# solonas13/REAL

Hardware: AMD Instinct MI355X
Metric: aligned reads/sec (100 bp, k≤3) at 1/2/4/8 MI355X; achieved HBM GB/s vs peak (higher is better)
Workload: dtype u64

## Files before the change

### real_amd/csrc/index_build.hip

```cpp
#include "real_hip_internal.h"

#include <cstring>
#include <rocprim/device/device_radix_sort.hpp>
#include <rocprim/device/device_scan.hpp>
#include <rocprim/iterator/transform_iterator.hpp>
#include <rocprim/device/device_select.hpp>
#include <rocprim/iterator/counting_iterator.hpp>

__global__ void pack_text_kernel(const uint8_t *__restrict__ sym, uint64_t n, uint64_t *__restrict__ text,
                                 uint64_t *__restrict__ wild, unsigned long long *n_wild)
{
    uint64_t w = (uint64_t)blockIdx.x * blockDim.x + threadIdx.x;
    uint64_t base = w * 64;
    if (base >= n) return;
    uint64_t t0 = 0, t1 = 0, wd = 0;
    for (int b = 0; b < 64; ++b) {
        uint64_t i = base + b;
        if (i < n) {
            uint64_t c = sym[i];
            if (c > 3) wd |= 1ull << (63 - b);
            c &= 3;
            if (b < 32) t0 |= c << (62 - 2 * b); else t1 |= c << (62 - 2 * (b - 32));
        }
    }
// ... 213 lines not shown
        if (!complex_ && c > 15) {
            uint32_t cnt[16];
            bucket_groups(ent, start, end, pbits, fbits >= 32 ? 15u : (1u << fbits) - 1, cnt);
#pragma unroll
            for (int g = 0; g < 16; ++g) complex_ = complex_ || cnt[g] > 15;
        }
        out = complex_ ? c : 0u;
    }
    ovf_cnt[p] = out;
}

__global__ void rows_fill_kernel(const uint32_t *__restrict__ bkt, const uint2 *__restrict__ ent, uint64_t nbuckets, uint32_t pbits,
                                 uint32_t fbits, const uint32_t *__restrict__ ovf_start, uint4 *__restrict__ rows, uint2 *__restrict__ ovf)
{
    const uint64_t p = (uint64_t)blockIdx.x * blockDim.x + threadIdx.x;
    if (p >= nbuckets) return;
    const uint32_t start = bkt[p], end = bkt[p + 1], c = end - start;
    const uint32_t os = ovf_start[p], oc = ovf_start[p + 1] - os;
    uint32_t w[32];
#pragma unroll
    for (int i = 0; i < 32; ++i) w[i] = 0;
    uint32_t cnt[16];
    bucket_groups(ent, start, end, pbits, fbits >= 32 ? 15u : (1u << fbits) - 1, cnt);
    if (oc) {
        rh_row_set_complex(w, os, c);
#pragma unroll
        for (int g = 0; g < 16; ++g) rh_row_set_count8(w, g, cnt[g]);
        for (uint32_t j = 0; j < c; ++j) ovf[os + j] = ent[start + j];
    } else {
#pragma unroll
        for (int g = 0; g < 16; ++g) rh_row_set_count4(w, g, cnt[g]);
        const uint32_t p16 = pbits < 16 ? pbits : 16;
        const uint32_t pmask = pbits ? ((1u << pbits) - 1) : 0u;
        for (uint32_t j = 0; j < c; ++j) {
            const uint2 e = ent[start + j];
            const uint32_t key = pbits ? ((e.x & pmask) >> (pbits - p16)) : rh_fp16(e.x);
            const uint32_t hw[3] = {key & 0xffffu, e.y & 0xffffu, e.y >> 16};
#pragma unroll
            for (int t = 0; t < 3; ++t) {
                const uint32_t h = rh_row_entry_hw(j) + t;
                const uint32_t v = hw[t] << (16 * (h & 1));
#pragma unroll
                for (int i = 2; i < 32; ++i) if ((h >> 1) == (uint32_t)i) w[i] |= v;
            }
        }
    }
#pragma unroll
    for (int i = 0; i < 8; ++i) rows[p * 8 + i] = make_uint4(w[4 * i], w[4 * i + 1], w[4 * i + 2], w[4 * i + 3]);
}

__device__ __forceinline__ uint32_t row_entries(uint32_t h0, uint32_t h1, uint32_t w3) { return rh_row_complex(h0, h1) ? w3 : rh_row_group4(h0, h1, 16).x; }

__global__ void pair_overflow_kernel(const uint32_t *__restrict__ bkt, const uint2 *__restrict__ ent, uint64_t nbuckets, uint32_t pbits,
                                     uint32_t gbits, const uint4 *__restrict__ rows, uint32_t *__restrict__ ovf_cnt)
{
    const uint64_t p = (uint64_t)blockIdx.x * blockDim.x + threadIdx.x;
    if (p > nbuckets) return;
    uint32_t out = 0;
    if (p < nbuckets) {
        const uint4 h = rows[p * 8];
        const uint32_t ca = row_entries(h.x, h.y, h.w);
        const uint32_t start = bkt[p], end = bkt[p + 1], c = end - start;
        bool complex_ = rh_row_complex(h.x, h.y) || ca + c > RH_ROW_CAP;
        if (!complex_ && c > 15) {
            uint32_t cnt[16];
            bucket_groups(ent, start, end, pbits, (1u << gbits) - 1, cnt);
#pragma unroll
            for (int g = 0; g < 16; ++g) complex_ = complex_ || cnt[g] > 15;
        }
        out = complex_ ? ca + c : 0u;
    }
    ovf_cnt[p] = out;
}

__global__ void pair_fill_kernel(const uint32_t *__restrict__ bkt, const uint2 *__restrict__ ent, uint64_t nbuckets, uint32_t pbits,
                                 uint32_t gbits, const uint32_t *__restrict__ ovf_start, uint32_t *rows, const uint2 *__restrict__ first_ovf,
                                 uint2 *__restrict__ ovf, const uint64_t *__restrict__ T, uint32_t l, int first_list)
{
// ... 4 lines not shown
    if (!c && !oc) return;
    uint32_t *w = rows + p * 32;
    const uint32_t h0 = w[0], h1 = w[1];
    const bool first_complex = rh_row_complex(h0, h1);
    const uint32_t ca = row_entries(h0, h1, w[3]);
    uint32_t cnt[16];
    bucket_groups(ent, start, end, pbits, (1u << gbits) - 1, cnt);
    if (oc) {
        uint32_t hd[8] = {0, 0, 0, 0, 0, 0, 0, 0};
        rh_row_set_complex(hd, os, ca + c);
        if (first_complex) {
            const uint32_t fo = w[2];
            for (int i = 4; i < 8; ++i) hd[i] = w[i];
            for (uint32_t j = 0; j < ca; ++j) ovf[os + j] = first_ovf[fo + j];
        } else {
            uint32_t j = 0;
            for (uint32_t g = 0; g < 16; ++g) {
                const uint32_t cg = rh_row_group4(h0, h1, g).y;
                rh_row_set_count8(hd, g, cg);
                for (uint32_t i = 0; i < cg; ++i, ++j) {
                    const uint32_t wp = rh_row_entry(w, j).y;
                    const uint32_t partner = (uint32_t)(window_signature(T, wp, l, 5 - first_list) >> (l - pbits));
                    ovf[os + j] = make_uint2((g << pbits) | partner, wp);
                }
            }
        }
        for (uint32_t g = 0; g < 16; ++g) if (cnt[g]) rh_row_set_count8(hd, g, cnt[g]);
        for (uint32_t j = 0; j < c; ++j) ovf[os + ca + j] = ent[start + j];
        for (int i = 0; i < 32; ++i) w[i] = i < 8 ? hd[i] : 0u;
    } else {
        uint32_t hd[2] = {h0, h1};
        for (uint32_t g = 0; g < 16; ++g) rh_row_set_count4(hd, g, cnt[g]);
        w[0] = hd[0]; w[1] = hd[1];
        uint16_t *hw = reinterpret_cast<uint16_t *>(w);
        const uint32_t p16 = pbits < 16 ? pbits : 16, pmask = (1u << pbits) - 1;
        for (uint32_t j = 0; j < c; ++j) {
            const uint2 e = ent[start + j];
            const uint32_t h = rh_row_entry_hw(ca + j);
            hw[h] = (uint16_t)((e.x & pmask) >> (pbits - p16)); hw[h + 1] = (uint16_t)(e.y & 0xffffu); hw[h + 2] = (uint16_t)(e.y >> 16);
        }
    }
}

__device__ __forceinline__ uint32_t ovf_groups_below(const uint2 *__restrict__ ovf, uint32_t o0, uint32_t tot, uint32_t pbits, uint32_t g)
{
    if (g == 0) return 0;
    if (g >= 16) return tot;
    uint32_t x = 0, y = tot;
    while (x < y) { const uint32_t mid = x + ((y - x) >> 1); if ((ovf[o0 + mid].x >> pbits) < g) x = mid + 1; else y = mid; }
    return x;
}
__global__ void rows_sizes_kernel(const uint4 *__restrict__ rows, const uint2 *__restrict__ ovf, uint64_t nbuckets, uint32_t pbits, uint32_t g0,
                                  uint32_t g1, uint32_t *__restrict__ size)
{
    const uint64_t p = (uint64_t)blockIdx.x * blockDim.x + threadIdx.x;
    if (p > nbuckets) return;
    uint32_t c = 0;
    if (p < nbuckets) {
        const uint4 h = rows[p * 8];
        c = rh_row_complex(h.x, h.y) ? ovf_groups_below(ovf, h.z, h.w, pbits, g1) - ovf_groups_below(ovf, h.z, h.w, pbits, g0)
                                     : rh_row_group4(h.x, h.y, g1).x - rh_row_group4(h.x, h.y, g0).x;
    }
    size[p] = c;
}
__global__ void rows_unpack_kernel(const uint4 *__restrict__ rows, const uint2 *__restrict__ ovf, uint64_t nbuckets, uint32_t pbits, uint32_t g0,
                                   const uint32_t *__restrict__ off, uint2 *__restrict__ out)
{
    const uint64_t p = (uint64_t)blockIdx.x * blockDim.x + threadIdx.x;
    if (p >= nbuckets) return;
    const uint32_t *w = reinterpret_cast<const uint32_t *>(rows + p * 8);
    const uint32_t o = off[p], c = off[p + 1] - o;
    if (rh_row_complex(w[0], w[1])) {
// ... 658 lines not shown
```

### real_amd/csrc/match_kernel.hip

```cpp
#include "match_common.h"

#ifndef RH_ABLATE
#define RH_ABLATE 0
#endif
#ifndef RH_PHASE_TIMING
#define RH_PHASE_TIMING 0
#endif

#if RH_PHASE_TIMING
#define PH_NOW() ((unsigned)__builtin_amdgcn_s_memrealtime())
#else
#define PH_NOW() 0u
#endif
#define EB 8
#define MQ 16
#define QUEUE_BYTES (MQ * 64u * 5u + 6u * 64u * 4u)
enum : int { TK_STARTS = 0, TK_DIRECTORY = 1, TK_ROWS = 3, TK_ROWS_WIDE = 4 };
__host__ __device__ constexpr uint32_t stg_bytes(int W, int TK) { return TK >= TK_ROWS ? 11008u : (W <= 4 ? QUEUE_BYTES : 9728u); }
#define MQR 8u
static_assert(MQR == RH_QSPILL_SLOTS, "the spill area holds a second queue of MQR slots per lane");
#define NPEND2 24
#define MQR2 24u
#define STG_PAD 16u
#ifndef RH_KEEP_TW_MAXW
// ... 572 lines not shown
{
    const uintptr_t a0 = (uintptr_t)src, a1 = a0 + nbytes, c0 = a0 & ~(uintptr_t)15;
    for (uintptr_t c = c0 + 16u * lane; c < a1; c += 16u * 64u) {
        const uint32_t lo = STG_PAD + (uint32_t)(c - c0);
        if (c >= a0 && c + 16 <= a1) {
            *reinterpret_cast<uint4 *>(stg + lo) = *reinterpret_cast<const uint4 *>(c);
        } else {
            for (int b = 0; b < 16; ++b)
                if (c + b >= a0 && c + b < a1) stg[lo + b] = *reinterpret_cast<const uint8_t *>(c + b);
        }
    }
    return STG_PAD + (uint32_t)(a0 - c0);
}
__device__ __forceinline__ void wave_lds_sync()
{
    __builtin_amdgcn_fence(__ATOMIC_SEQ_CST, "wavefront");
    __builtin_amdgcn_wave_barrier();
}

template <class T>
__device__ __forceinline__ bool quals_ahead(const MatchArgs &a, uint64_t o0, uint64_t o1, const uint8_t *&src, uint32_t &nbytes, uint32_t &late, uint32_t &skew)
{
    if (!a.b.qual || a.b.gl < 64) return false;
    const uint64_t gb = __shfl(o0, 0), ge = __shfl(o1, 63);
    skew = (uint32_t)((uintptr_t)(a.b.qual + gb) & 15u);
    src = a.b.qual + gb - skew;
    nbytes = (uint32_t)(ge - gb) + skew;
    late = nbytes <= 64u * 128u ? 0u : T::ROWBUF - STG_PAD;
    return ge >= gb && gb >= skew && ge - gb + skew <= T::STG_CAP;
}
template <class T>
__device__ __forceinline__ uint32_t quals_at(uint32_t late, uint32_t skew) { return (late ? STG_PAD : T::ROWBUF) + skew; }

__device__ __forceinline__ void quals_landed()
{
    asm volatile("s_waitcnt vmcnt(0)" ::: "memory");
}

template <class T, int LA0, int LA1>
__device__ __forceinline__ void match_lists_rows(const MatchArgs &a, LaneState<T> &s, const double *sLL, uint8_t *stg, bool act, bool qlast)
{
    constexpr bool wide = T::WIDE;
    constexpr int NL = LA1 - LA0;
    uint32_t lane = threadIdx.x & 63;
    asm volatile("" : "+v"(lane));
    uint32_t *q_pos = reinterpret_cast<uint32_t *>(stg) + lane;
    uint8_t *q_la = stg + T::QSLOTS * 64 * 4 + lane;
    uint8_t *rowbuf = stg + T::ROWBUF;
    const uint32_t bb = a.b_bits;
    const uint32_t gbits = a.ix.fbits, pbits = a.ix.pbits, p16 = pbits < 16 ? pbits : 16;
    const uint32_t pmask = (1u << pbits) - 1;
    uint64_t M = 0, MA = 0, MB = 0;
    if (!wide) {
        const uint32_t mb = (1u << bb) - 1;
        M = ((uint64_t)(uint32_t)(s.shi >> bb) << 48) | ((uint64_t)((uint32_t)s.shi & mb) << 32) | ((uint64_t)(uint32_t)(s.slo >> bb) << 16) |
            (uint64_t)((uint32_t)s.slo & mb);
    } else {
        const uint64_t mb = (bb >= 32) ? 0xffffffffull : ((1ull << bb) - 1);
        MA = ((s.shi >> bb) << 32) | (s.shi & mb);
        MB = ((s.slo >> bb) << 32) | (s.slo & mb);
    }
    auto sig_of = [&](int la) {
        const uint2 x = rh_list_segs(la);
        return (((uint32_t)(M >> (48 - 16 * x.x)) & 0xffffu) << bb) | ((uint32_t)(M >> (48 - 16 * x.y)) & 0xffffu);
    };
    auto sig_wide = [&](int la) {
// ... 104 lines not shown
                    if ((g >> 2) == (uint32_t)q) e_cnt = (w >> (8 * (g & 3))) & 255u;
                    const uint32_t y = ~w | ~upto;
                    sat255 |= (y - 0x01010101u) & ~y & 0x80808080u;
                }
                const bool sat = sat255 != 0;
                const uint32_t o0 = row(2), tot = row(3);
                e_base = o0 + off;
                if (sat) {
                    const uint2 kr = key_group_range(a.ix.ent[la], o0, o0 + tot, wide ? 28u : pbits, g);
                    e_base = kr.x; e_cnt = kr.y;
                }
            }
            if (!wide) s.addC(e_cnt);
            s.addP(e_cnt);
            if (e_cnt > T::BIG) { s.p_n = PEND_OVF; s.cslot = (!T::PASS2 && T::HAS_PASS2 && e_cnt <= BIG_T2) ? SLOT_NONE : SLOT_BIG; e_cnt = 0; }
            if (RH_ABLATE & 4) e_cnt = 0;
        }
        const uint32_t rk = wide ? rh_fp16(r) : (r >> (pbits - p16));
        U64x2 pre = {0ull, 0ull};
        if (e_ovf && e_cnt) pre = load2(reinterpret_cast<const uint64_t *>(a.ix.ent[la] + e_base));
        if (li + 1 < NL) ISSUE_ROWS(la + 1);
        auto take = [&](bool pass, uint32_t pos) {
            const bool merge = pass && qn && pos == q_last;
            if ((!wide || T::DEFER) && pass && !merge && qn >= 2) {
                for (uint32_t k = 0; k + 1 < qn; ++k)
                    if (q_pos[k * 64] == pos) { q_la[k * 64] |= (uint8_t)(1u << la); pass = false; break; }
            }
            if (pass && !merge && qn == T::QSLOTS) { s.p_n = PEND_OVF; e_cnt = 0; pass = false; }
            const uint32_t slot = merge ? qn - 1 : qn;
            const uint32_t lav = (merge ? q_lastla : 0u) | (1u << la);
            if (pass) { q_pos[slot * 64] = pos; q_la[slot * 64] = (uint8_t)lav; q_last = pos; q_lastla = lav; qn = slot + 1; }
        };
        auto passes = [&](uint32_t x) { return wide ? (x == 0u) : (__popc(((x >> 1) | x) & 0x55555555u) <= a.seedkmax); };
        uint32_t passm = 0;
        while (__any(!e_ovf && e_j < e_cnt)) {
#pragma unroll
            for (uint32_t u = 0; u < 4; ++u) {
                const uint32_t jj = e_j + u;
                const bool ok = !e_ovf && jj < e_cnt;
                const uint32_t h = ok ? rh_row_entry_hw(e_base + jj) : 4u;
                const uint32_t d0 = row(h >> 1);
                const uint32_t key = (h & 1) ? (d0 >> 16) : (d0 & 0xffffu);
                passm |= (ok && passes(key ^ rk) ? 1u : 0u) << (jj & 31u);
            }
            e_j += 4;
        }
        if (!T::PASS2 && T::HAS_PASS2 && __popc(passm) > NPEND) { s.p_n = PEND_OVF; passm = 0; e_cnt = 0; }
        while (__any(passm != 0)) {
            const bool step = passm != 0;
            const uint32_t jj = step ? (uint32_t)__ffs((int)passm) - 1u : 0u;
            passm &= passm - 1u;
            const uint32_t h = step ? rh_row_entry_hw(e_base + jj) : 4u;
            const uint32_t d0 = row(h >> 1), d1 = row((h >> 1) + 1);
            take(step, (h & 1) ? d1 : ((d0 >> 16) | (d1 << 16)));
        }
        auto take_ovf = [&](bool ok, uint2 e) { take(ok && passes(wide ? (e.x ^ r) : ((e.x & pmask) ^ r)), e.y); };
        if (__any(e_ovf && e_cnt)) {
            take_ovf(e_ovf && e_cnt > 0, make_uint2((uint32_t)pre.a, (uint32_t)(pre.a >> 32)));
            take_ovf(e_ovf && e_cnt > 1, make_uint2((uint32_t)pre.b, (uint32_t)(pre.b >> 32)));
        }
        e_j = 2;
        while (__any(e_ovf && e_j < e_cnt)) {
            uint2 e[T::OVN];
#pragma unroll
            for (uint32_t u = 0; u < T::OVN; ++u) e[u] = (e_ovf && e_j + u < e_cnt) ? a.ix.ent[la][e_base + e_j + u] : make_uint2(0u, 0u);
#pragma unroll
            for (uint32_t u = 0; u < T::OVN; ++u) take_ovf(e_ovf && e_j + u < e_cnt, e[u]);
            e_j += T::OVN;
        }
#if RH_PHASE_TIMING
        s.tD += PH_NOW() - ph1;
#endif
    }
    if (T::SCORES && qlast) ISSUE_QUALS();
#if RH_PHASE_TIMING
    const unsigned ph2 = PH_NOW();
#endif
    if (s.p_n == PEND_OVF) qn = 0;
    {
        CandText<T::W> c0;
        uint32_t rp0 = qn ? q_pos[0] : 0u;
        if (qn) cand_load(a, s, rp0, c0);
        for (uint32_t k = 0; k < qn; ++k) {
            CandText<T::W> c1;
            uint32_t rp1 = 0;
            if (k + 1 < qn) { rp1 = q_pos[(k + 1) * 64]; cand_load(a, s, rp1, c1); }
            process_loaded(a, s, sLL, rp0, (uint32_t)q_la[k * 64], c0);
            c0 = c1; rp0 = rp1;
        }
    }
#if RH_PHASE_TIMING
    s.tR += PH_NOW() - ph2;
#endif
    if (T::SCORES && qlast) ISSUE_QUALS_LATE();
#undef ISSUE_QUALS
#undef ISSUE_QUALS_LATE
#undef QUAL_DMA
}

template <class T>
__device__ __forceinline__ void match_rows_paired(const MatchArgs &a, LaneState<T> &s, const double *sLL, uint8_t *stg, bool act, uint32_t rhi,
                                                  uint32_t rlo)
{
    constexpr uint32_t QS = T::QSLOTS;
    uint32_t lane = threadIdx.x & 63;
    asm volatile("" : "+v"(lane));
    uint32_t *q_pos = reinterpret_cast<uint32_t *>(stg) + lane;
    uint8_t *q_la = stg + QS * 64 * 4 + lane;
    uint8_t *rowbuf = stg + T::ROWBUF;
    auto spill = [&](uint32_t k) -> uint2 & { return a.qspill[((size_t)(blockIdx.x * 4u + (threadIdx.x >> 6)) * QS + (k - QS)) * 64u + lane]; };
    const uint32_t bb = a.b_bits;
    const uint32_t gbits = a.ix.fbits, pbits = a.ix.pbits, p16 = pbits < 16 ? pbits : 16;
    const uint32_t pmask = (1u << pbits) - 1;
    const uint32_t mb = (1u << bb) - 1, fhi = (uint32_t)s.shi, flo = (uint32_t)s.slo;
    auto sig_of = [&](uint32_t strand, uint32_t la) {
        const uint32_t hi = strand ? rhi : fhi, lo = strand ? rlo : flo;
        const uint2 x = rh_list_segs(la);
        const uint32_t sa_ = ((x.x < 2 ? hi : lo) >> ((x.x & 1) ? 0u : bb)) & mb, sc_ = ((x.y < 2 ? hi : lo) >> ((x.y & 1) ? 0u : bb)) & mb;
        return (sa_ << bb) | sc_;
    };
    auto row_of = [&](uint32_t li) { return rh_row_addr(li >> 1, sig_of(li & 1u, li >> 1), a.l, gbits).row; };
    uint32_t qn = 0, qnf = 0, q_last = 0, q_lastla = 0;
    auto q_getp = [&](uint32_t k) { return k < QS ? q_pos[k * 64] : spill(k).x; };
    auto q_getl = [&](uint32_t k) { return k < QS ? (uint32_t)q_la[k * 64] : spill(k).y; };
    uint4 va0, va1, va2, va3, va4, va5, va6, va7;
    uint32_t *bkx = reinterpret_cast<uint32_t *>(stg + T::BKX);
#define ISSUE_ROWS_P(LI)                                                                                                    \
    do {                                                                                                                    \
        bkx[(lane & 7) * 8 + (lane >> 3)] = act ? row_of(LI) : 0u;                                                          \
        __builtin_amdgcn_wave_barrier();                                                                                    \
        const uint4 b0_ = *reinterpret_cast<const uint4 *>(bkx + (lane >> 3) * 8);                                          \
        const uint4 b1_ = *reinterpret_cast<const uint4 *>(bkx + (lane >> 3) * 8 + 4);                                      \
        const uint4 *__restrict__ R_ = reinterpret_cast<const uint4 *>(a.ix.bkt[(LI) >> 1]) + (lane & 7);                   \
        va0 = R_[(uint64_t)b0_.x * 8]; va1 = R_[(uint64_t)b0_.y * 8]; va2 = R_[(uint64_t)b0_.z * 8];                        \
        va3 = R_[(uint64_t)b0_.w * 8]; va4 = R_[(uint64_t)b1_.x * 8]; va5 = R_[(uint64_t)b1_.y * 8];                        \
        va6 = R_[(uint64_t)b1_.z * 8]; va7 = R_[(uint64_t)b1_.w * 8];                                                       \
    } while (0)
#define QUAL_DMA(SRC_OFF, LDS_ADDR, NBYTES, NCHUNK)                                                                                           \
    _Pragma("unroll") for (uint32_t i = 0; i < (NCHUNK); ++i)                                                                                 \
        if (16u * lane + 1024u * i + 16u <= (NBYTES)) {                                                                                       \
            const uint8_t *g_ = qsrc + (SRC_OFF) + 16u * lane + 1024u * i;                                                                    \
            uint32_t keep_;                                                                                                                   \
            asm volatile("s_mov_b32 %0, m0\n\ts_mov_b32 m0, %2\n\ts_nop 0\n\tglobal_load_lds_dwordx4 %1, off\n\ts_mov_b32 m0, %0"         \
                         : "=&s"(keep_) : "v"(g_), "s"((LDS_ADDR) + 1024u * i) : "memory");                                                   \
        }
    ISSUE_ROWS_P(0u);
#pragma unroll 1
    for (uint32_t li = 0; li < 8; ++li) {
        const uint32_t tbl = li >> 1, ks = li & 1u;
#if RH_PHASE_TIMING
        const unsigned ph0 = PH_NOW();
#endif
        wave_lds_sync();
        {
            uint8_t *d = rowbuf + (lane >> 3) * 128 + (((lane & 7) ^ ((lane >> 3) & 7)) * 16);
            *reinterpret_cast<uint4 *>(d + 0 * 1024) = va0; *reinterpret_cast<uint4 *>(d + 1 * 1024) = va1;
            *reinterpret_cast<uint4 *>(d + 2 * 1024) = va2; *reinterpret_cast<uint4 *>(d + 3 * 1024) = va3;
            *reinterpret_cast<uint4 *>(d + 4 * 1024) = va4; *reinterpret_cast<uint4 *>(d + 5 * 1024) = va5;
            *reinterpret_cast<uint4 *>(d + 6 * 1024) = va6; *reinterpret_cast<uint4 *>(d + 7 * 1024) = va7;
        }
        wave_lds_sync();
#if RH_PHASE_TIMING
        unsigned ph1 = PH_NOW();
        s.tW += ph1 - ph0;
#endif
        const uint8_t *rowb = rowbuf + lane * 128;
        const uint32_t sw = lane & 7;
        auto row = [&](uint32_t d) { return *reinterpret_cast<const uint32_t *>(rowb + ((((d >> 2) ^ sw) << 4) | ((d & 3) << 2))); };
        const RhRowAddr ra = rh_row_addr(tbl, sig_of(ks, tbl), a.l, gbits);
        const uint32_t nhalf = tbl < 2 ? 2u : 1u;
#pragma unroll 1
        for (uint32_t half = 0; half < nhalf; ++half) {
            const uint32_t strand = ks ^ half, la = half ? 5 - tbl : tbl;
            const uint32_t g = ra.group | (half << (gbits - 1));
            const uint32_t r = sig_of(strand, 5 - la) >> (a.l - pbits);
            const bool mine = act && !(s.p_n == PEND_OVF) && !(RH_ABLATE & 8);
            uint32_t e_cnt = 0, e_j = 0, e_base = 0;
            bool e_ovf = false;
            if (mine) {
                s.addL(1u);
                const uint32_t h0 = row(0), h1 = row(1);
                if (!rh_row_complex(h0, h1)) {
                    e_cnt = ((g < 8 ? h0 : h1) >> (4 * (g & 7))) & 15u;
                    const uint32_t m0 = g < 8 ? (g ? (h0 & (0xffffffffu >> (32 - 4 * g))) : 0u) : h0;
                    const uint32_t m1 = g > 8 ? (h1 & (0xffffffffu >> (32 - 4 * (g - 8)))) : 0u;
                    const uint32_t b0 = (m0 & 0x0f0f0f0fu) + ((m0 >> 4) & 0x0f0f0f0fu), b1 = (m1 & 0x0f0f0f0fu) + ((m1 >> 4) & 0x0f0f0f0fu);
                    e_base = __builtin_amdgcn_sad_u8(b0, 0u, __builtin_amdgcn_sad_u8(b1, 0u, 0u));
                } else {
                    e_ovf = true;
                    uint32_t off = 0, sat255 = 0;
#pragma unroll
                    for (int q = 0; q < 4; ++q) {
                        const uint32_t w = row(4 + q);
                        const int nb = (int)g - 4 * q;
                        const uint32_t below = nb <= 0 ? 0u : (nb >= 4 ? 0xffffffffu : ((1u << (8 * nb)) - 1u));
                        const uint32_t upto = nb < 0 ? 0u : (nb >= 3 ? 0xffffffffu : ((1u << (8 * (nb + 1))) - 1u));
                        off = __builtin_amdgcn_sad_u8(w & below, 0u, off);
                        if ((g >> 2) == (uint32_t)q) e_cnt = (w >> (8 * (g & 3))) & 255u;
                        const uint32_t y = ~w | ~upto;
                        sat255 |= (y - 0x01010101u) & ~y & 0x80808080u;
                    }
                    const uint32_t o0 = row(2), tot = row(3);
                    e_base = o0 + off;
                    if (sat255 != 0) {
                        const uint2 kr = key_group_range(a.ix.ent[tbl], o0, o0 + tot, pbits, g);
                        e_base = kr.x; e_cnt = kr.y;
                    }
                }
                s.addC(e_cnt);
                s.addP(e_cnt);
                if (e_cnt > T::BIG) { s.p_n = PEND_OVF; s.cslot = e_cnt <= BIG_T2 ? SLOT_NONE : SLOT_BIG; e_cnt = 0; }
                if (RH_ABLATE & 4) e_cnt = 0;
            }
            U64x2 pre = {0ull, 0ull};
            if (e_ovf && e_cnt) pre = load2(reinterpret_cast<const uint64_t *>(a.ix.ent[tbl] + e_base));
            if (half == 0 && li + 1 < 8) ISSUE_ROWS_P(li + 1);
            auto take = [&](bool pass, uint32_t pos) {
                const bool merge = pass && qn && pos == q_last && (q_lastla >> 6) == strand;
                if (pass && !merge && qn >= 2) {
                    for (uint32_t k = 0; k + 1 < qn; ++k)
                        if (q_getp(k) == pos && (q_getl(k) >> 6) == strand) {
                            if (k < QS) q_la[k * 64] |= (uint8_t)(1u << la); else spill(k).y |= 1u << la;
                            pass = false; break;
                        }
                }
                if (pass && !merge && (strand ? qn - qnf : qnf) == QS) { s.p_n = PEND_OVF; e_cnt = 0; pass = false; }
                const uint32_t slot = merge ? qn - 1 : qn;
                const uint32_t lav = (merge ? q_lastla : (strand << 6)) | (1u << la);
                if (pass) {
                    if (slot < QS) { q_pos[slot * 64] = pos; q_la[slot * 64] = (uint8_t)lav; } else spill(slot) = make_uint2(pos, lav);
                    q_last = pos; q_lastla = lav; qn = slot + 1;
                    if (!merge && !strand) qnf++;
                }
            };
            auto passes = [&](uint32_t x) { return __popc(((x >> 1) | x) & 0x55555555u) <= a.seedkmax; };
            uint32_t passm = 0;
            while (__any(!e_ovf && e_j < e_cnt)) {
#pragma unroll
                for (uint32_t u = 0; u < 4; ++u) {
                    const uint32_t jj = e_j + u;
                    const bool ok = !e_ovf && jj < e_cnt;
                    const uint32_t h = ok ? rh_row_entry_hw(e_base + jj) : 4u;
                    const uint32_t d0 = row(h >> 1);
                    const uint32_t key = (h & 1) ? (d0 >> 16) : (d0 & 0xffffu);
                    passm |= (ok && passes(key ^ (r >> (pbits - p16))) ? 1u : 0u) << (jj & 31u);
                }
                e_j += 4;
            }
            if (__popc(passm) > NPEND) { s.p_n = PEND_OVF; passm = 0; e_cnt = 0; }
            while (__any(passm != 0)) {
                const bool step = passm != 0;
                const uint32_t jj = step ? (uint32_t)__ffs((int)passm) - 1u : 0u;
                passm &= passm - 1u;
                const uint32_t h = step ? rh_row_entry_hw(e_base + jj) : 4u;
                const uint32_t d0 = row(h >> 1), d1 = row((h >> 1) + 1);
                take(step, (h & 1) ? d1 : ((d0 >> 16) | (d1 << 16)));
            }
            auto take_ovf = [&](bool ok, uint2 e) { take(ok && passes((e.x & pmask) ^ r), e.y); };
            if (__any(e_ovf && e_cnt)) {
                take_ovf(e_ovf && e_cnt > 0, make_uint2((uint32_t)pre.a, (uint32_t)(pre.a >> 32)));
                take_ovf(e_ovf && e_cnt > 1, make_uint2((uint32_t)pre.b, (uint32_t)(pre.b >> 32)));
            }
            e_j = 2;
            while (__any(e_ovf && e_j < e_cnt)) {
                uint2 e[T::OVN];
#pragma unroll
                for (uint32_t u = 0; u < T::OVN; ++u) e[u] = (e_ovf && e_j + u < e_cnt) ? a.ix.ent[tbl][e_base + e_j + u] : make_uint2(0u, 0u);
#pragma unroll
                for (uint32_t u = 0; u < T::OVN; ++u) take_ovf(e_ovf && e_j + u < e_cnt, e[u]);
                e_j += T::OVN;
            }
        }
#if RH_PHASE_TIMING
        s.tD += PH_NOW() - ph1;
#endif
    }
    const uint32_t patl = act ? s.patl : 32u * T::W;
#pragma unroll 1
    for (uint32_t inv = 0; inv < 2; ++inv) {
        if (inv && act) {
            uint64_t R[T::W];
            revcomp_words<T::W>(s.O, R, patl);
#pragma unroll
            for (int j = 0; j < T::W; ++j) s.O[j] = R[j];
        }
        s.shi = inv ? rhi : fhi; s.slo = inv ? rlo : flo;
        s.reset_strand((int)inv);
        if (T::SCORES && inv) {
            const uint8_t *qsrc;
            uint32_t qbytes, qlate, qskew;
            if (quals_ahead<T>(a, s.o0, s.o1, qsrc, qbytes, qlate, qskew)) {
// ... 321 lines not shown
```

### real_amd/csrc/real_hip_internal.h

```cpp
#pragma once

#include <hip/hip_runtime.h>
#include <stdint.h>
#include <string>
#include <vector>

#include "real_hip.h"

#define RH_MAXW 10
static_assert(RH_MAXW * 32 == REAL_HIP_MAX_PATL, "one lane-per-read instance per 32 bases up to REAL_HIP_MAX_PATL");
#define RH_CSTRIPES 1024
#define RH_QSPILL_SLOTS 8u

struct DevText {
    const uint64_t *text;
    const uint64_t *wild;
    const uint64_t *frag_start;
    uint64_t n;
    uint32_t n_frag;
    uint32_t has_wild;
    uint32_t fileid;
};

enum RhLayout : uint32_t { RH_LAYOUT_STARTS = 0, RH_LAYOUT_DIGEST = 1, RH_LAYOUT_FINGERPRINT = 2, RH_LAYOUT_ROWS = 3 };
// ... 18 lines not shown
#define RH_FP_SLOTS 8u
static inline __host__ __device__ uint32_t rh_fp11(uint32_t key) { return (key * 0x9E3779B1u) >> 21; }

static inline __host__ __device__ uint2 key_group_range(const uint2 *E, uint32_t lo, uint32_t hi, uint32_t shift, uint32_t key)
{
    uint32_t x = lo, y = hi;
    while (x < y) { const uint32_t mid = x + ((y - x) >> 1); if ((E[mid].x >> shift) < key) x = mid + 1; else y = mid; }
    const uint32_t first = x;
    for (y = hi; x < y;) { const uint32_t mid = x + ((y - x) >> 1); if ((E[mid].x >> shift) <= key) x = mid + 1; else y = mid; }
    return make_uint2(first, x - first);
}

#define RH_ROW_CAP 20u
#define RH_ROW_SAT 255u
static inline __host__ __device__ uint32_t rh_fp16(uint32_t key) { return ((key & 0x0fffffffu) * 0x9E3779B1u) >> 16; }
static inline __host__ __device__ bool rh_row_complex(uint32_t h0, uint32_t h1) { return (h0 & h1) == 0xffffffffu; }
static inline __host__ __device__ uint2 rh_row_group4(uint32_t h0, uint32_t h1, uint32_t g)
{
    uint32_t base = 0, cnt = 0;
    for (uint32_t q = 0; q < 16; ++q) { const uint32_t c = ((q < 8 ? h0 : h1) >> (4 * (q & 7))) & 15u; if (q < g) base += c; if (q == g) cnt = c; }
    return make_uint2(base, cnt);
}
static inline __host__ __device__ uint2 rh_row_group8(const uint32_t *row, uint32_t g, bool *sat)
{
    uint32_t base = 0, cnt = 0;
    bool s = false;
    for (uint32_t q = 0; q <= g; ++q) { const uint32_t c = (row[4 + (q >> 2)] >> (8 * (q & 3))) & 255u; s = s || c == RH_ROW_SAT; if (q < g) base += c; else cnt = c; }
    *sat = s;
    return make_uint2(base, cnt);
}
static inline __host__ __device__ void rh_row_set_complex(uint32_t *w, uint32_t first, uint32_t total) { w[0] = w[1] = 0xffffffffu; w[2] = first; w[3] = total; }
static inline __host__ __device__ void rh_row_set_count4(uint32_t *w, uint32_t g, uint32_t c) { w[g >> 3] |= c << (4 * (g & 7)); }
static inline __host__ __device__ void rh_row_set_count8(uint32_t *w, uint32_t g, uint32_t c) { w[4 + (g >> 2)] |= (c < RH_ROW_SAT ? c : RH_ROW_SAT) << (8 * (g & 3)); }
static inline __host__ __device__ uint32_t rh_row_entry_hw(uint32_t j) { return 4 + 3 * j; }
static inline __host__ __device__ uint2 rh_row_entry(const uint32_t *row, uint32_t j)
{
    const uint32_t h = rh_row_entry_hw(j);
    const uint32_t d0 = row[h >> 1], d1 = row[(h >> 1) + 1];
    return make_uint2((h & 1) ? (d0 >> 16) : (d0 & 0xffffu), (h & 1) ? d1 : ((d0 >> 16) | (d1 << 16)));
}

#include "row_addr.h"

static inline void rh_index_geometry(uint32_t l, uint32_t pb, uint32_t *pshift, uint32_t *fshift, uint32_t *fbits, uint32_t *pbits)
{
    const uint32_t R = l - pb;
    *pshift = R;
    if (R <= 30) {
        uint32_t pbts = (32 - R) & ~1u;
        if (pbts > l) pbts = l;
        if (pbts > 30) pbts = 30;
        *fshift = 0; *fbits = R; *pbits = pbts;
    } else {
        *fshift = R - 32; *fbits = 32; *pbits = 0;
    }
}

struct DevBatch {
    const uint8_t  *bases;
    const uint8_t  *qual;
    const uint64_t *off;
    uint64_t n_reads;
    uint32_t upatl;
    uint32_t W;
    uint32_t gl;
    uint32_t packed;
    const uint8_t *nflags;
    uint32_t fresh;
    uint32_t maxpatl;
};

struct MatchArgs {
// ... 150 lines not shown
```

### real_amd/csrc/row_addr.h

```cpp
#pragma once
#include <stdint.h>
#if defined(__HIPCC__)
#define RH_HD __host__ __device__
#else
#define RH_HD
#endif

#define RH_MIX32 0x9E3779B1u
#define RH_MIX64 0x9E3779B97F4A7C15ull
static inline RH_HD uint32_t rh_mix32(uint32_t sign, uint32_t l) { return (sign * RH_MIX32) & (l >= 32 ? 0xffffffffu : ((1u << l) - 1u)); }
static inline RH_HD uint64_t rh_mix64(uint64_t sign, uint32_t l) { return (sign * RH_MIX64) & (l >= 64 ? ~0ull : ((1ull << l) - 1ull)); }

static inline RH_HD bool rh_list_paired(uint32_t la) { return la < 2 || la > 3; }
static inline RH_HD uint32_t rh_sig_rcform(uint32_t sign, uint32_t l)
{
    uint32_t x = sign;
    x = ((x >> 2) & 0x33333333u) | ((x & 0x33333333u) << 2);
    x = ((x >> 4) & 0x0f0f0f0fu) | ((x & 0x0f0f0f0fu) << 4);
    x = ((x >> 8) & 0x00ff00ffu) | ((x & 0x00ff00ffu) << 8);
    x = (x >> 16) | (x << 16);
    return ~x >> (32 - l);
}
static inline RH_HD uint32_t rh_place_sig(uint32_t la, uint32_t sign, uint32_t l) { return la > 3 ? rh_sig_rcform(sign, l) : sign; }
struct RhRowAddr { uint32_t table, row, group; };
static inline RH_HD RhRowAddr rh_row_addr(uint32_t la, uint32_t sign, uint32_t l, uint32_t gbits)
{
    const uint32_t mixed = rh_mix32(rh_place_sig(la, sign, l), l);
    if (!rh_list_paired(la)) return {la, mixed >> gbits, mixed & ((1u << gbits) - 1u)};
    const uint32_t h = gbits - 1;
    return {la > 3 ? 5 - la : la, mixed >> h, ((la > 3 ? 1u : 0u) << h) | (mixed & ((1u << h) - 1u))};
}
static inline RH_HD uint64_t rh_table_rows(uint32_t la, uint32_t l, uint32_t pb) { return (l <= 32 && rh_list_paired(la)) ? 2ull << pb : 1ull << pb; }
```

### real_amd/csrc/kernel_common.h

```cpp
#pragma once
#include "real_hip_internal.h"

#define M55 0x5555555555555555ull

__device__ __forceinline__ unsigned pairdiff(uint64_t x) { return __popcll(((x >> 1) | x) & M55); }

__device__ __forceinline__ uint64_t text_bits(const uint64_t *__restrict__ T, uint64_t i, unsigned nb)
{
    uint64_t w = i >> 5;
    unsigned sh = 2u * (unsigned)(i & 31);
    uint64_t v = T[w] << sh;
    if (sh + 2 * nb > 64) v |= T[w + 1] >> (64 - sh);
    return v >> (64 - 2 * nb);
}

__device__ __forceinline__ bool frag_valid(const DevText &t, uint32_t pos, uint32_t patl, uint32_t &frag)
{
    if (t.n_frag == 1) {
        frag = 0;
        return (uint64_t)pos + patl <= t.n;
    }
    uint32_t lo = 0, hi = t.n_frag + 1;
    while (lo < hi) {
        uint32_t mid = (lo + hi) >> 1;
        if (t.frag_start[mid] <= (uint64_t)pos) lo = mid + 1; else hi = mid;
    }
    frag = lo - 1;
    return (uint64_t)pos + patl <= t.frag_start[lo];
}

__device__ __forceinline__ bool wild_free(const uint64_t *__restrict__ Wd, uint32_t pos, uint32_t patl)
{
    uint64_t a = pos, e = (uint64_t)pos + patl - 1;
    uint64_t wa = a >> 6, we = e >> 6;
    for (uint64_t w = wa; w <= we; ++w) {
        uint64_t m = ~0ull;
        if (w == wa) m &= ~0ull >> (a & 63);
        if (w == we) m &= ~0ull << (63 - (e & 63));
// ... 86 lines not shown
```

Before: 4.085 billion.

## Split row entries into packed key array and dword-aligned position array

Row entries in the hash index change from interleaved 3-halfword records to two separate arrays: one of 16-bit keys and one of 32-bit positions. The build kernels and the row accessors are updated to match. The match kernel now filters two keys per dword load through a new row_filter helper and fetches each position with one aligned read instead of two reads plus a shift. It also computes the mixed signature once and reuses it for row addressing, which relies on that cached value matching the table being probed.

```diff
diff --git a/real_amd/csrc/index_build.hip b/real_amd/csrc/index_build.hip
--- a/real_amd/csrc/index_build.hip
+++ b/real_amd/csrc/index_build.hip
@@ -269,18 +269,12 @@
         for (int g = 0; g < 16; ++g) rh_row_set_count4(w, g, cnt[g]);
         const uint32_t p16 = pbits < 16 ? pbits : 16;
         const uint32_t pmask = pbits ? ((1u << pbits) - 1) : 0u;
-        for (uint32_t j = 0; j < c; ++j) {
-            const uint2 e = ent[start + j];
-            const uint32_t key = pbits ? ((e.x & pmask) >> (pbits - p16)) : rh_fp16(e.x);
-            const uint32_t hw[3] = {key & 0xffffu, e.y & 0xffffu, e.y >> 16};
-#pragma unroll
-            for (int t = 0; t < 3; ++t) {
-                const uint32_t h = rh_row_entry_hw(j) + t;
-                const uint32_t v = hw[t] << (16 * (h & 1));
-#pragma unroll
-                for (int i = 2; i < 32; ++i) if ((h >> 1) == (uint32_t)i) w[i] |= v;
+#pragma unroll
+        for (uint32_t j = 0; j < RH_ROW_CAP; ++j)
+            if (j < c) {
+                const uint2 e = ent[start + j];
+                rh_row_set_entry(w, j, pbits ? ((e.x & pmask) >> (pbits - p16)) : rh_fp16(e.x), e.y);
             }
-        }
     }
 #pragma unroll
     for (int i = 0; i < 8; ++i) rows[p * 8 + i] = make_uint4(w[4 * i], w[4 * i + 1], w[4 * i + 2], w[4 * i + 3]);
@@ -351,12 +345,12 @@
         uint32_t hd[2] = {h0, h1};
         for (uint32_t g = 0; g < 16; ++g) rh_row_set_count4(hd, g, cnt[g]);
         w[0] = hd[0]; w[1] = hd[1];
+        const uint32_t p16 = pbits < 16 ? pbits : 16, pmask = (1u << pbits) - 1;
         uint16_t *hw = reinterpret_cast<uint16_t *>(w);
-        const uint32_t p16 = pbits < 16 ? pbits : 16, pmask = (1u << pbits) - 1;
         for (uint32_t j = 0; j < c; ++j) {
             const uint2 e = ent[start + j];
-            const uint32_t h = rh_row_entry_hw(ca + j);
-            hw[h] = (uint16_t)((e.x & pmask) >> (pbits - p16)); hw[h + 1] = (uint16_t)(e.y & 0xffffu); hw[h + 2] = (uint16_t)(e.y >> 16);
+            hw[rh_row_key_hw(ca + j)] = (uint16_t)((e.x & pmask) >> (pbits - p16));
+            w[rh_row_pos_dw(ca + j)] = e.y;
         }
     }
 }
diff --git a/real_amd/csrc/match_kernel.hip b/real_amd/csrc/match_kernel.hip
--- a/real_amd/csrc/match_kernel.hip
+++ b/real_amd/csrc/match_kernel.hip
@@ -628,6 +628,31 @@
 template <class T>
 __device__ __forceinline__ uint32_t quals_at(uint32_t late, uint32_t skew) { return (late ? STG_PAD : T::ROWBUF) + skew; }
 
+template <bool WIDE, class Row>
+__device__ __forceinline__ uint32_t row_filter(Row row, bool simple, uint32_t e_base, uint32_t e_cnt, uint32_t rk, uint32_t seedkmax)
+{
+    const bool go = simple && e_cnt;
+    const uint32_t h = rh_row_key_hw(go ? e_base : 0u);
+    const uint32_t odd = h & 1u;
+    const uint32_t need = go ? e_cnt + odd : 0u;
+    const uint32_t rk2 = rk | (rk << 16);
+    uint32_t d = h >> 1, acc = 0;
+    for (uint32_t cov = 0; __any(cov < need); cov += 6, d += 3) {
+#pragma unroll
+        for (uint32_t u = 0; u < 3; ++u) {
+            const uint32_t x = row(d + u) ^ rk2;
+            bool lo, hi;
+            if (WIDE) { lo = (x & 0xffffu) == 0u; hi = (x >> 16) == 0u; }
+            else {
+                const uint32_t m = ((x >> 1) | x) & 0x55555555u;
+                lo = (uint32_t)__popc(m & 0xffffu) <= seedkmax; hi = (uint32_t)__popc(m >> 16) <= seedkmax;
+            }
+            acc |= ((lo ? 1u : 0u) | (hi ? 2u : 0u)) << (cov + 2u * u);
+        }
+    }
+    return go ? (acc >> odd) & ((1u << e_cnt) - 1u) : 0u;
+}
+
 __device__ __forceinline__ void quals_landed()
 {
     asm volatile("s_waitcnt vmcnt(0)" ::: "memory");
@@ -798,27 +823,13 @@
             if (pass) { q_pos[slot * 64] = pos; q_la[slot * 64] = (uint8_t)lav; q_last = pos; q_lastla = lav; qn = slot + 1; }
         };
         auto passes = [&](uint32_t x) { return wide ? (x == 0u) : (__popc(((x >> 1) | x) & 0x55555555u) <= a.seedkmax); };
-        uint32_t passm = 0;
-        while (__any(!e_ovf && e_j < e_cnt)) {
-#pragma unroll
-            for (uint32_t u = 0; u < 4; ++u) {
-                const uint32_t jj = e_j + u;
-                const bool ok = !e_ovf && jj < e_cnt;
-                const uint32_t h = ok ? rh_row_entry_hw(e_base + jj) : 4u;
-                const uint32_t d0 = row(h >> 1);
-                const uint32_t key = (h & 1) ? (d0 >> 16) : (d0 & 0xffffu);
-                passm |= (ok && passes(key ^ rk) ? 1u : 0u) << (jj & 31u);
-            }
-            e_j += 4;
-        }
+        uint32_t passm = row_filter<wide>(row, !e_ovf, e_base, e_cnt, rk, a.seedkmax);
         if (!T::PASS2 && T::HAS_PASS2 && __popc(passm) > NPEND) { s.p_n = PEND_OVF; passm = 0; e_cnt = 0; }
         while (__any(passm != 0)) {
             const bool step = passm != 0;
             const uint32_t jj = step ? (uint32_t)__ffs((int)passm) - 1u : 0u;
             passm &= passm - 1u;
-            const uint32_t h = step ? rh_row_entry_hw(e_base + jj) : 4u;
-            const uint32_t d0 = row(h >> 1), d1 = row((h >> 1) + 1);
-            take(step, (h & 1) ? d1 : ((d0 >> 16) | (d1 << 16)));
+            take(step, row(rh_row_pos_dw(step ? e_base + jj : 0u)));
         }
         auto take_ovf = [&](bool ok, uint2 e) { take(ok && passes(wide ? (e.x ^ r) : ((e.x & pmask) ^ r)), e.y); };
         if (__any(e_ovf && e_cnt)) {
@@ -885,7 +896,8 @@
         const uint32_t sa_ = ((x.x < 2 ? hi : lo) >> ((x.x & 1) ? 0u : bb)) & mb, sc_ = ((x.y < 2 ? hi : lo) >> ((x.y & 1) ? 0u : bb)) & mb;
         return (sa_ << bb) | sc_;
     };
-    auto row_of = [&](uint32_t li) { return rh_row_addr(li >> 1, sig_of(li & 1u, li >> 1), a.l, gbits).row; };
+    auto mixed_of = [&](uint32_t li) { return rh_mix32(sig_of(li & 1u, li >> 1), a.l); };
+    uint32_t mx = 0;
     uint32_t qn = 0, qnf = 0, q_last = 0, q_lastla = 0;
     auto q_getp = [&](uint32_t k) { return k < QS ? q_pos[k * 64] : spill(k).x; };
     auto q_getl = [&](uint32_t k) { return k < QS ? (uint32_t)q_la[k * 64] : spill(k).y; };
@@ -893,7 +905,8 @@
     uint32_t *bkx = reinterpret_cast<uint32_t *>(stg + T::BKX);
 #define ISSUE_ROWS_P(LI)                                                                                                    \
     do {                                                                                                                    \
-        bkx[(lane & 7) * 8 + (lane >> 3)] = act ? row_of(LI) : 0u;                                                          \
+        mx = mixed_of(LI);                                                                                                  \
+        bkx[(lane & 7) * 8 + (lane >> 3)] = act ? rh_row_addr_mixed((LI) >> 1, mx, gbits).row : 0u;                         \
         __builtin_amdgcn_wave_barrier();                                                                                    \
         const uint4 b0_ = *reinterpret_cast<const uint4 *>(bkx + (lane >> 3) * 8);                                          \
         const uint4 b1_ = *reinterpret_cast<const uint4 *>(bkx + (lane >> 3) * 8 + 4);                                      \
@@ -933,7 +946,7 @@
         const uint8_t *rowb = rowbuf + lane * 128;
         const uint32_t sw = lane & 7;
         auto row = [&](uint32_t d) { return *reinterpret_cast<const uint32_t *>(rowb + ((((d >> 2) ^ sw) << 4) | ((d & 3) << 2))); };
-        const RhRowAddr ra = rh_row_addr(tbl, sig_of(ks, tbl), a.l, gbits);
+        const RhRowAddr ra = rh_row_addr_mixed(tbl, mx, gbits);
         const uint32_t nhalf = tbl < 2 ? 2u : 1u;
 #pragma unroll 1
         for (uint32_t half = 0; half < nhalf; ++half) {
@@ -1000,27 +1013,13 @@
                 }
             };
             auto passes = [&](uint32_t x) { return __popc(((x >> 1) | x) & 0x55555555u) <= a.seedkmax; };
-            uint32_t passm = 0;
-            while (__any(!e_ovf && e_j < e_cnt)) {
-#pragma unroll
-                for (uint32_t u = 0; u < 4; ++u) {
-                    const uint32_t jj = e_j + u;
-                    const bool ok = !e_ovf && jj < e_cnt;
-                    const uint32_t h = ok ? rh_row_entry_hw(e_base + jj) : 4u;
-                    const uint32_t d0 = row(h >> 1);
-                    const uint32_t key = (h & 1) ? (d0 >> 16) : (d0 & 0xffffu);
-                    passm |= (ok && passes(key ^ (r >> (pbits - p16))) ? 1u : 0u) << (jj & 31u);
-                }
-                e_j += 4;
-            }
+            uint32_t passm = row_filter<false>(row, !e_ovf, e_base, e_cnt, r >> (pbits - p16), a.seedkmax);
             if (__popc(passm) > NPEND) { s.p_n = PEND_OVF; passm = 0; e_cnt = 0; }
             while (__any(passm != 0)) {
                 const bool step = passm != 0;
                 const uint32_t jj = step ? (uint32_t)__ffs((int)passm) - 1u : 0u;
                 passm &= passm - 1u;
-                const uint32_t h = step ? rh_row_entry_hw(e_base + jj) : 4u;
-                const uint32_t d0 = row(h >> 1), d1 = row((h >> 1) + 1);
-                take(step, (h & 1) ? d1 : ((d0 >> 16) | (d1 << 16)));
+                take(step, row(rh_row_pos_dw(step ? e_base + jj : 0u)));
             }
             auto take_ovf = [&](bool ok, uint2 e) { take(ok && passes((e.x & pmask) ^ r), e.y); };
             if (__any(e_ovf && e_cnt)) {
diff --git a/real_amd/csrc/real_hip_internal.h b/real_amd/csrc/real_hip_internal.h
--- a/real_amd/csrc/real_hip_internal.h
+++ b/real_amd/csrc/real_hip_internal.h
@@ -74,12 +74,19 @@
 static inline __host__ __device__ void rh_row_set_complex(uint32_t *w, uint32_t first, uint32_t total) { w[0] = w[1] = 0xffffffffu; w[2] = first; w[3] = total; }
 static inline __host__ __device__ void rh_row_set_count4(uint32_t *w, uint32_t g, uint32_t c) { w[g >> 3] |= c << (4 * (g & 7)); }
 static inline __host__ __device__ void rh_row_set_count8(uint32_t *w, uint32_t g, uint32_t c) { w[4 + (g >> 2)] |= (c < RH_ROW_SAT ? c : RH_ROW_SAT) << (8 * (g & 3)); }
-static inline __host__ __device__ uint32_t rh_row_entry_hw(uint32_t j) { return 4 + 3 * j; }
+static inline __host__ __device__ uint32_t rh_row_key_hw(uint32_t j) { return 4 + j; }
+static inline __host__ __device__ uint32_t rh_row_pos_dw(uint32_t j) { return 12 + j; }
+static_assert(2 * 12 == 4 + RH_ROW_CAP && 12 + RH_ROW_CAP == 32, "a simple row: header, RH_ROW_CAP keys, RH_ROW_CAP positions fill the 32 words");
 static inline __host__ __device__ uint2 rh_row_entry(const uint32_t *row, uint32_t j)
 {
-    const uint32_t h = rh_row_entry_hw(j);
-    const uint32_t d0 = row[h >> 1], d1 = row[(h >> 1) + 1];
-    return make_uint2((h & 1) ? (d0 >> 16) : (d0 & 0xffffu), (h & 1) ? d1 : ((d0 >> 16) | (d1 << 16)));
+    const uint32_t h = rh_row_key_hw(j);
+    return make_uint2((row[h >> 1] >> (16 * (h & 1))) & 0xffffu, row[rh_row_pos_dw(j)]);
+}
+static inline __host__ __device__ void rh_row_set_entry(uint32_t *w, uint32_t j, uint32_t key, uint32_t pos)
+{
+    const uint32_t h = rh_row_key_hw(j);
+    w[h >> 1] |= (key & 0xffffu) << (16 * (h & 1));
+    w[rh_row_pos_dw(j)] = pos;
 }
 
 #include "row_addr.h"
diff --git a/real_amd/csrc/row_addr.h b/real_amd/csrc/row_addr.h
--- a/real_amd/csrc/row_addr.h
+++ b/real_amd/csrc/row_addr.h
@@ -23,11 +23,14 @@
 }
 static inline RH_HD uint32_t rh_place_sig(uint32_t la, uint32_t sign, uint32_t l) { return la > 3 ? rh_sig_rcform(sign, l) : sign; }
 struct RhRowAddr { uint32_t table, row, group; };
-static inline RH_HD RhRowAddr rh_row_addr(uint32_t la, uint32_t sign, uint32_t l, uint32_t gbits)
+static inline RH_HD RhRowAddr rh_row_addr_mixed(uint32_t la, uint32_t mixed, uint32_t gbits)
 {
-    const uint32_t mixed = rh_mix32(rh_place_sig(la, sign, l), l);
     if (!rh_list_paired(la)) return {la, mixed >> gbits, mixed & ((1u << gbits) - 1u)};
     const uint32_t h = gbits - 1;
     return {la > 3 ? 5 - la : la, mixed >> h, ((la > 3 ? 1u : 0u) << h) | (mixed & ((1u << h) - 1u))};
 }
+static inline RH_HD RhRowAddr rh_row_addr(uint32_t la, uint32_t sign, uint32_t l, uint32_t gbits)
+{
+    return rh_row_addr_mixed(la, rh_mix32(rh_place_sig(la, sign, l), l), gbits);
+}
 static inline RH_HD uint64_t rh_table_rows(uint32_t la, uint32_t l, uint32_t pb) { return (l <= 32 && rh_list_paired(la)) ? 2ull << pb : 1ull << pb; }
```

After: 4.265 billion, median of 6. 4.4% higher.

## Scan both strand groups of simple rows in one pass using udot8 offsets

Applied to the files above, without the earlier changes.

For simple (non-overflow) hash rows, both strand groups' entry counts and base offsets are now computed once up front, with udot8 nibble dot products replacing the masked byte-sum and SAD sequence. Both groups' candidates are filtered and queued in a single combined scan loop, and the second half-iteration runs only when some lane in the wave has a complex row. This is meant to cut loop overhead, wave-divergent iterations and redundant row reads in the seed lookup phase. It adds a combined mask word that assumes the row cap is below 32, and it changes how pending-list overflow is checked per group.

```diff
diff --git a/real_amd/csrc/kernel_common.h b/real_amd/csrc/kernel_common.h
--- a/real_amd/csrc/kernel_common.h
+++ b/real_amd/csrc/kernel_common.h
@@ -4,6 +4,7 @@
 #define M55 0x5555555555555555ull
 
 __device__ __forceinline__ unsigned pairdiff(uint64_t x) { return __popcll(((x >> 1) | x) & M55); }
+__device__ __forceinline__ uint32_t nibble_dot(uint32_t x, uint32_t w, uint32_t acc) { return __builtin_amdgcn_udot8(x, w, acc, false); }
 
 __device__ __forceinline__ uint64_t text_bits(const uint64_t *__restrict__ T, uint64_t i, unsigned nb)
 {
diff --git a/real_amd/csrc/match_kernel.hip b/real_amd/csrc/match_kernel.hip
--- a/real_amd/csrc/match_kernel.hip
+++ b/real_amd/csrc/match_kernel.hip
@@ -934,44 +934,76 @@
         const uint32_t sw = lane & 7;
         auto row = [&](uint32_t d) { return *reinterpret_cast<const uint32_t *>(rowb + ((((d >> 2) ^ sw) << 4) | ((d & 3) << 2))); };
         const RhRowAddr ra = rh_row_addr(tbl, sig_of(ks, tbl), a.l, gbits);
-        const uint32_t nhalf = tbl < 2 ? 2u : 1u;
+        const bool pairt = tbl < 2;
+        const uint32_t g0 = ra.group, g1 = pairt ? g0 | (1u << (gbits - 1)) : g0;
+        const uint32_t r0 = sig_of(ks, 5 - tbl) >> (a.l - pbits);
+        const uint32_t r1 = pairt ? sig_of(ks ^ 1u, tbl) >> (a.l - pbits) : 0u;
+        const bool mine = act && !(s.p_n == PEND_OVF) && !(RH_ABLATE & 8);
+        const uint32_t h0 = row(0), h1 = row(1);
+        const bool cplx = mine && rh_row_complex(h0, h1);
+        uint32_t c0 = 0, c1 = 0, eb0 = 0, eb1 = 0;
+        if (mine && !cplx) {
+            const uint64_t hh = ((uint64_t)h1 << 32) | h0, ones = 0x1111111111111111ull;
+            const uint64_t below0 = ones & ~(~0ull << (4 * g0));
+            eb0 = nibble_dot(h0, (uint32_t)below0, nibble_dot(h1, (uint32_t)(below0 >> 32), 0u));
+            c0 = (uint32_t)(hh >> (4 * g0)) & 15u;
+            if (pairt) {
+                const uint64_t ext = (ones & ~(~0ull << (4 * g1))) ^ below0;
+                eb1 = nibble_dot(h0, (uint32_t)ext, nibble_dot(h1, (uint32_t)(ext >> 32), eb0));
+                c1 = (uint32_t)(hh >> (4 * g1)) & 15u;
+            }
+            s.addL(pairt ? 2u : 1u);
+            s.addC(c0 + c1);
+            s.addP(c0 + c1);
+            if (RH_ABLATE & 4) c0 = c1 = 0;
+        }
+        uint32_t e_cnt = 0;
+        auto take = [&](bool pass, uint32_t pos, uint32_t strand, uint32_t la) {
+            const bool merge = pass && qn && pos == q_last && (q_lastla >> 6) == strand;
+            if (pass && !merge && qn >= 2) {
+                for (uint32_t k = 0; k + 1 < qn; ++k)
+                    if (q_getp(k) == pos && (q_getl(k) >> 6) == strand) {
+                        if (k < QS) q_la[k * 64] |= (uint8_t)(1u << la); else spill(k).y |= 1u << la;
+                        pass = false; break;
+                    }
+            }
+            if (pass && !merge && (strand ? qn - qnf : qnf) == QS) { s.p_n = PEND_OVF; e_cnt = 0; pass = false; }
+            const uint32_t slot = merge ? qn - 1 : qn;
+            const uint32_t lav = (merge ? q_lastla : (strand << 6)) | (1u << la);
+            if (pass) {
+                if (slot < QS) { q_pos[slot * 64] = pos; q_la[slot * 64] = (uint8_t)lav; } else spill(slot) = make_uint2(pos, lav);
+                q_last = pos; q_lastla = lav; qn = slot + 1;
+                if (!merge && !strand) qnf++;
+            }
+        };
+        auto passes = [&](uint32_t x) { return __popc(((x >> 1) | x) & 0x55555555u) <= a.seedkmax; };
+        const uint32_t nhalf = (pairt && __any(cplx)) ? 2u : 1u;
 #pragma unroll 1
         for (uint32_t half = 0; half < nhalf; ++half) {
             const uint32_t strand = ks ^ half, la = half ? 5 - tbl : tbl;
-            const uint32_t g = ra.group | (half << (gbits - 1));
-            const uint32_t r = sig_of(strand, 5 - la) >> (a.l - pbits);
-            const bool mine = act && !(s.p_n == PEND_OVF) && !(RH_ABLATE & 8);
-            uint32_t e_cnt = 0, e_j = 0, e_base = 0;
-            bool e_ovf = false;
-            if (mine) {
+            const uint32_t g = half ? g1 : g0, r = half ? r1 : r0;
+            const bool e_ovf = cplx && !(s.p_n == PEND_OVF);
+            uint32_t e_j = 0, e_base = 0;
+            e_cnt = 0;
+            if (e_ovf) {
                 s.addL(1u);
-                const uint32_t h0 = row(0), h1 = row(1);
-                if (!rh_row_complex(h0, h1)) {
-                    e_cnt = ((g < 8 ? h0 : h1) >> (4 * (g & 7))) & 15u;
-                    const uint32_t m0 = g < 8 ? (g ? (h0 & (0xffffffffu >> (32 - 4 * g))) : 0u) : h0;
-                    const uint32_t m1 = g > 8 ? (h1 & (0xffffffffu >> (32 - 4 * (g - 8)))) : 0u;
-                    const uint32_t b0 = (m0 & 0x0f0f0f0fu) + ((m0 >> 4) & 0x0f0f0f0fu), b1 = (m1 & 0x0f0f0f0fu) + ((m1 >> 4) & 0x0f0f0f0fu);
-                    e_base = __builtin_amdgcn_sad_u8(b0, 0u, __builtin_amdgcn_sad_u8(b1, 0u, 0u));
-                } else {
-                    e_ovf = true;
-                    uint32_t off = 0, sat255 = 0;
-#pragma unroll
-                    for (int q = 0; q < 4; ++q) {
-                        const uint32_t w = row(4 + q);
-                        const int nb = (int)g - 4 * q;
-                        const uint32_t below = nb <= 0 ? 0u : (nb >= 4 ? 0xffffffffu : ((1u << (8 * nb)) - 1u));
-                        const uint32_t upto = nb < 0 ? 0u : (nb >= 3 ? 0xffffffffu : ((1u << (8 * (nb + 1))) - 1u));
-                        off = __builtin_amdgcn_sad_u8(w & below, 0u, off);
-                        if ((g >> 2) == (uint32_t)q) e_cnt = (w >> (8 * (g & 3))) & 255u;
-                        const uint32_t y = ~w | ~upto;
-                        sat255 |= (y - 0x01010101u) & ~y & 0x80808080u;
-                    }
-                    const uint32_t o0 = row(2), tot = row(3);
-                    e_base = o0 + off;
-                    if (sat255 != 0) {
-                        const uint2 kr = key_group_range(a.ix.ent[tbl], o0, o0 + tot, pbits, g);
-                        e_base = kr.x; e_cnt = kr.y;
-                    }
+                uint32_t off = 0, sat255 = 0;
+#pragma unroll
+                for (int q = 0; q < 4; ++q) {
+                    const uint32_t w = row(4 + q);
+                    const int nb = (int)g - 4 * q;
+                    const uint32_t below = nb <= 0 ? 0u : (nb >= 4 ? 0xffffffffu : ((1u << (8 * nb)) - 1u));
+                    const uint32_t upto = nb < 0 ? 0u : (nb >= 3 ? 0xffffffffu : ((1u << (8 * (nb + 1))) - 1u));
+                    off = __builtin_amdgcn_sad_u8(w & below, 0u, off);
+                    if ((g >> 2) == (uint32_t)q) e_cnt = (w >> (8 * (g & 3))) & 255u;
+                    const uint32_t y = ~w | ~upto;
+                    sat255 |= (y - 0x01010101u) & ~y & 0x80808080u;
+                }
+                const uint32_t o0 = row(2), tot = row(3);
+                e_base = o0 + off;
+                if (sat255 != 0) {
+                    const uint2 kr = key_group_range(a.ix.ent[tbl], o0, o0 + tot, pbits, g);
+                    e_base = kr.x; e_cnt = kr.y;
                 }
                 s.addC(e_cnt);
                 s.addP(e_cnt);
@@ -980,49 +1012,37 @@
             }
             U64x2 pre = {0ull, 0ull};
             if (e_ovf && e_cnt) pre = load2(reinterpret_cast<const uint64_t *>(a.ix.ent[tbl] + e_base));
-            if (half == 0 && li + 1 < 8) ISSUE_ROWS_P(li + 1);
-            auto take = [&](bool pass, uint32_t pos) {
-                const bool merge = pass && qn && pos == q_last && (q_lastla >> 6) == strand;
-                if (pass && !merge && qn >= 2) {
-                    for (uint32_t k = 0; k + 1 < qn; ++k)
-                        if (q_getp(k) == pos && (q_getl(k) >> 6) == strand) {
-                            if (k < QS) q_la[k * 64] |= (uint8_t)(1u << la); else spill(k).y |= 1u << la;
-                            pass = false; break;
-                        }
+            if (half == 0) {
+                if (li + 1 < 8) ISSUE_ROWS_P(li + 1);
+                static_assert(RH_ROW_CAP < 32, "one mask word for both groups of a simple row");
+                const uint32_t ct = c0 + c1, d1 = eb1 - c0;
+                const uint32_t rk0 = r0 >> (pbits - p16), rk1 = r1 >> (pbits - p16);
+                uint32_t passm = 0;
+                while (__any(e_j < ct)) {
+#pragma unroll
+                    for (uint32_t u = 0; u < 4; ++u) {
+                        const uint32_t jj = e_j + u;
+                        const bool ok = jj < ct, sec = jj >= c0;
+                        const uint32_t h = ok ? rh_row_entry_hw(jj + (sec ? d1 : eb0)) : 4u;
+                        const uint32_t d0 = row(h >> 1);
+                        const uint32_t key = (h & 1) ? (d0 >> 16) : (d0 & 0xffffu);
+                        passm |= (ok && passes(key ^ (sec ? rk1 : rk0)) ? 1u : 0u) << (jj & 31u);
+                    }
+                    e_j += 4;
                 }
-                if (pass && !merge && (strand ? qn - qnf : qnf) == QS) { s.p_n = PEND_OVF; e_cnt = 0; pass = false; }
-                const uint32_t slot = merge ? qn - 1 : qn;
-                const uint32_t lav = (merge ? q_lastla : (strand << 6)) | (1u << la);
-                if (pass) {
-                    if (slot < QS) { q_pos[slot * 64] = pos; q_la[slot * 64] = (uint8_t)lav; } else spill(slot) = make_uint2(pos, lav);
-                    q_last = pos; q_lastla = lav; qn = slot + 1;
-                    if (!merge && !strand) qnf++;
+                const uint32_t low = (1u << c0) - 1u;
+                if (__popc(passm & low) > NPEND || __popc(passm & ~low) > NPEND) { s.p_n = PEND_OVF; passm = 0; }
+                while (__any(passm != 0)) {
+                    const bool step = passm != 0;
+                    const uint32_t jj = step ? (uint32_t)__ffs((int)passm) - 1u : 0u;
+                    passm &= passm - 1u;
+                    const bool sec = jj >= c0;
+                    const uint32_t h = step ? rh_row_entry_hw(jj + (sec ? d1 : eb0)) : 4u;
+                    const uint32_t d0 = row(h >> 1), d1w = row((h >> 1) + 1);
+                    take(step, (h & 1) ? d1w : ((d0 >> 16) | (d1w << 16)), ks ^ (sec ? 1u : 0u), sec ? 5 - tbl : tbl);
                 }
-            };
-            auto passes = [&](uint32_t x) { return __popc(((x >> 1) | x) & 0x55555555u) <= a.seedkmax; };
-            uint32_t passm = 0;
-            while (__any(!e_ovf && e_j < e_cnt)) {
-#pragma unroll
-                for (uint32_t u = 0; u < 4; ++u) {
-                    const uint32_t jj = e_j + u;
-                    const bool ok = !e_ovf && jj < e_cnt;
-                    const uint32_t h = ok ? rh_row_entry_hw(e_base + jj) : 4u;
-                    const uint32_t d0 = row(h >> 1);
-                    const uint32_t key = (h & 1) ? (d0 >> 16) : (d0 & 0xffffu);
-                    passm |= (ok && passes(key ^ (r >> (pbits - p16))) ? 1u : 0u) << (jj & 31u);
-                }
-                e_j += 4;
-            }
-            if (__popc(passm) > NPEND) { s.p_n = PEND_OVF; passm = 0; e_cnt = 0; }
-            while (__any(passm != 0)) {
-                const bool step = passm != 0;
-                const uint32_t jj = step ? (uint32_t)__ffs((int)passm) - 1u : 0u;
-                passm &= passm - 1u;
-                const uint32_t h = step ? rh_row_entry_hw(e_base + jj) : 4u;
-                const uint32_t d0 = row(h >> 1), d1 = row((h >> 1) + 1);
-                take(step, (h & 1) ? d1 : ((d0 >> 16) | (d1 << 16)));
-            }
-            auto take_ovf = [&](bool ok, uint2 e) { take(ok && passes((e.x & pmask) ^ r), e.y); };
+            }
+            auto take_ovf = [&](bool ok, uint2 e) { take(ok && passes((e.x & pmask) ^ r), e.y, strand, la); };
             if (__any(e_ovf && e_cnt)) {
                 take_ovf(e_ovf && e_cnt > 0, make_uint2((uint32_t)pre.a, (uint32_t)(pre.a >> 32)));
                 take_ovf(e_ovf && e_cnt > 1, make_uint2((uint32_t)pre.b, (uint32_t)(pre.b >> 32)));
```

Measured after the change: 4.058 billion before, 4.195 billion after (median of 6 runs). 1.03x the previous value.
